# melspectrum007/audio-visual-speech-enhancement

Measured on AMD Instinct MI355X. Metric: clips/sec (STFT+CNN forward) on 200-ms@16kHz segments, 1/2/4/8 MI355X, higher is better.
Workload: dtype fp32_split

## Files before the change

### audio-visual-speech-enhancement_amd/csrc/avse_common.h

```cpp
#pragma once
#include <hip/hip_runtime.h>
#include <stdint.h>
#include <string>

#include "forward_plan.h"
#include "ragged_geom.h"

typedef __bf16 bf16_t;
typedef __bf16 bf16x8 __attribute__((ext_vector_type(8)));
typedef _Float16 f16x8 __attribute__((ext_vector_type(8)));
typedef _Float16 f16x4 __attribute__((ext_vector_type(4)));
typedef float f32x4 __attribute__((ext_vector_type(4)));
typedef int i32x4 __attribute__((ext_vector_type(4)));

struct avse_ctx;

namespace avse {

void set_error(const std::string& msg);

int ctx_device_index(const struct ::avse_ctx* c);

int ensure_lds_attr(const void* fn, int bytes);

// ... 98 lines not shown
    int N;
    int hop;
    int n_mels;
    const float* pinvT;
    const float2* twiddle;
    const float* window;
    float* frames;
    float* sig;
    const float4* bins;
    const float* gram_inv;
};

int launch_istft(const IstftArgs& a, hipStream_t s);

int istft_ragged_chunk(int N, int hop, int n_mels, bool fused_tables);
int launch_istft_ragged(const IstftArgs& a, const RaggedGeom& g, const RaggedDev& d, hipStream_t s);

struct ConvArgs {
    const void* in;
    void* out;
    const void* w;
    const float* scale;
    const float* shift;
    const int2* taps;
    int N;
    int Hi, Wi, Ci;
    long long in_clip_stride;
    int Hq, Wq;
    int sy, sx;
    int oys, oxs;
    int Ho, Wo, Co;
    long long out_clip_stride;
    int out_pix_stride;
    int out_c_off;
    int pool;
    int act;
    int nphase;
    int ksplit;
    int ksplit_slabs;
    float* partial;
    const float* fuse_w;
    float fuse_bias;
    float* fuse_out;
    int out_s16;
    unsigned* range_flag;
    unsigned range_bit, range_in_bit;
    ConvPhase ph[MAX_PHASES];
};

__device__ __forceinline__ bool pair_out_of_range(float x) { return !(__builtin_fabsf(x) < 65520.f); }
__device__ __forceinline__ void range_report(unsigned* flag, unsigned bit, bool bad) {
    if (bad && flag) atomicOr(flag, bit);
}
constexpr unsigned kRangeAudioIn = 1u << 24, kRangeVideoIn = 1u << 25;
int launch_flag_or(unsigned* flag, unsigned bits, hipStream_t s);

constexpr int kConvSplit = 2, kConvSplitPairs = 3;
int launch_conv(const ConvArgs& a, int dtype, hipStream_t s);

int launch_conv_win(const ConvArgs& a, const int2* htaps, hipStream_t s);

struct DecTailArgs {
    const bf16_t* in;
    float* out;
    int N;
    const bf16_t* w4;
    const float* sc4;
    const float* sh4;
    int nt4, kpad4;
    int pt4, pl4, rows4, pitch4;
    int dy4, dx4, nx4;
    const bf16_t* w5;
    const float* sc5;
    const float* sh5;
    int nt5[4], kpad5[4];
    int dy5[4], dx5[4], nx5[4];
    long long woff5[4];
    int pt5, pl5, rows5, pitch5;
    const float* w6;
    float b6;
    unsigned* range_flag;
    unsigned range_bit;
    int four_products;
};
bool dec_tail_supported(const DecTailArgs& a);
bool dec_tail_s16_supported(const DecTailArgs& a);
int launch_dec_tail_s16(const DecTailArgs& a, hipStream_t s);

struct AudEncArgs {
    const float* mel;
    bf16_t* out;
    long long out_clip_stride;
    int N;
    const bf16_t* w1;
    const bf16_t* w2;
    const bf16_t* w3;
    const bf16_t* w4;
    const bf16_t* w5;
    const float* sc[5];
    const float* sh[5];
};
bool aud_enc_supported(const AudEncArgs& a);

struct DecHeadArgs {
    const bf16_t* in;
    long long in_clip_stride;
    bf16_t* out;
    long long out_clip_stride;
    int N;
    const bf16_t* w1;
    const bf16_t* w2;
    const bf16_t* w3;
    const float* sc[3];
    const float* sh[3];
};
bool dec_head_supported(const DecHeadArgs& a);
int launch_dec_head(const DecHeadArgs& a, hipStream_t s);

struct GemmArgs {
    const bf16_t* a;
    long long lda;
    const bf16_t* w;
    int M, N, kpad;
    const float* scale;
    const float* shift;
    int act;
    bf16_t* out;
    long long ldo;
    int out_off;
    int ksplit;
    float* partial;
    int* counters;
    int split;
    int slabs_per_split;
    unsigned* range_flag;
    unsigned range_bit;
    int counters_cap;
    int four_products;
};
int launch_gemm(const GemmArgs& g, int mode, hipStream_t s);
int launch_aud_enc(const AudEncArgs& a, hipStream_t s);
int launch_dec_tail(const DecTailArgs& a, hipStream_t s);

enum HaloOut { OUT_BF16 = 0, OUT_S16 = 1, OUT_F32 = 2 };

struct HaloArgs {
    int variant;
    const void* in;
    const float* video;
    const float* vmean;
    const float* vstd;
    void* out;
    const void* w;
    const float* scale;
    const float* shift;
    int N, Hc, Wc, Ci, Co;
    long long out_clip_stride;
    int out_pix_stride;
    int out_c_off;
    int mfma32;
    int no_planar;
    int split;
    int out_mode;
    unsigned long long* prof;
    unsigned* range_flag;
    unsigned range_bit, range_in_bit;
// ... 49 lines not shown
```

### audio-visual-speech-enhancement_amd/csrc/capi.hip

```cpp
#include <algorithm>
#include <cmath>
#include <cstdlib>
#include <cstring>
#include <mutex>
#include <set>

#include "ctx.h"
#include "eval_tables.h"
#include "spec_tables.h"

namespace avse {
static thread_local std::string g_err;
void set_error(const std::string& msg) { g_err = msg; }

int ensure_lds_attr(const void* fn, int bytes) {
    static std::mutex mu;
    static std::set<std::pair<const void*, int>> done;
    int dev = 0;
    AVSE_HIP_CHECK(hipGetDevice(&dev));
    std::lock_guard<std::mutex> lock(mu);
    if (done.count({fn, dev})) return 0;
    AVSE_HIP_CHECK(hipFuncSetAttribute(fn, hipFuncAttributeMaxDynamicSharedMemorySize, bytes));
    done.insert({fn, dev});
    return 0;
}

int fail(int code, const std::string& msg) {
    set_error(msg);
    return code;
}

int ctx_device_index(const avse_ctx* c) { return c->device; }
}

using namespace avse;

static_assert(sizeof(Cplx) == sizeof(float2) && offsetof(Cplx, im) == offsetof(float2, y), "Cplx must match float2");
static_assert(sizeof(MelBin) == sizeof(float4) && offsetof(MelBin, j0) == offsetof(float4, z), "MelBin must match float4");

struct OptionName {
    const char* name;
    const char* env;
    int Options::*field;
};
const OptionName kOptionNames[] = {
    {"no_gemm", "AVSE_NO_GEMM", &Options::no_gemm},
    {"no_audenc", "AVSE_NO_AUDENC", &Options::no_audenc},
    {"no_dechead", "AVSE_NO_DECHEAD", &Options::no_dechead},
    {"no_dectail", "AVSE_NO_DECTAIL", &Options::no_dectail},
    {"unfused_tail", "AVSE_UNFUSED_TAIL", &Options::unfused_tail},
    {"no_halo", "AVSE_NO_HALO", &Options::no_halo},
    {"mfma32", "AVSE_MFMA32", &Options::mfma32},
    {"serial", "AVSE_SERIAL", &Options::serial},
    {"graph", "AVSE_GRAPH", &Options::graph},
    {"gemm_ksplit_cap", "AVSE_GEMM_KSPLIT", &Options::gemm_ksplit_cap},
    {"dense_istft", "AVSE_DENSE_ISTFT", &Options::dense_istft},
    {"no_act_scale", "AVSE_NO_ACT_SCALE", &Options::no_act_scale},
    {"no_win", "AVSE_NO_WIN", &Options::no_win},
    {"no_v1p", "AVSE_NO_V1P", &Options::no_v1p},
    {"no_a1valu", "AVSE_NO_A1VALU", &Options::no_a1valu},
    {"no_planar", "AVSE_NO_PLANAR", &Options::no_planar},
    {"four_products", "AVSE_FOUR_PRODUCTS", &Options::four_products},
    {"side_prio", "AVSE_SIDE_PRIO", &Options::side_prio},
};

namespace {

const OptionName* find_option(const char* name) {
    for (const OptionName& o : kOptionNames)
        if (std::strcmp(o.name, name) == 0) return &o;
    return nullptr;
}

int upload_ragged(avse_ctx* c, const RaggedGeom& g, hipStream_t s, RaggedDev* d) {
    const size_t ub = sizeof(RaggedUtt) * g.utt.size(), ib = sizeof(RaggedItem) * g.items.size();
    const size_t need = ub + ib;
    hipStreamCaptureStatus cs = hipStreamCaptureStatusNone;
    if (s) AVSE_HIP_CHECK(hipStreamIsCapturing(s, &cs));
    const bool capturing = cs != hipStreamCaptureStatusNone;
    if (int rc = grow(c->prep, need, s, "preprocess scratch")) return rc;
    if (!capturing && c->ragged_done) AVSE_HIP_CHECK(hipEventSynchronize(c->ragged_done));
    if (int rc = grow(c->ragged_host, need, s, "ragged tables")) return rc;
    if (!c->ragged_done) AVSE_HIP_CHECK(hipEventCreateWithFlags(&c->ragged_done, hipEventDisableTiming));
    std::memcpy(c->ragged_host, g.utt.data(), ub);
    std::memcpy(c->ragged_host + ub, g.items.data(), ib);
    AVSE_HIP_CHECK(hipMemcpyAsync(c->prep, c->ragged_host, need, hipMemcpyHostToDevice, s));
    if (!capturing) AVSE_HIP_CHECK(hipEventRecord(c->ragged_done, s));
    d->utt = reinterpret_cast<const RaggedUtt*>(c->prep.p.get());
    d->items = reinterpret_cast<const RaggedItem*>(c->prep + ub);
    d->n_utt = (int)g.utt.size();
    d->n_items = (int)g.items.size();
    return 0;
}

template <typename D, typename T>
int table_to_device(const std::vector<T>& h, Owned<D>& out) {
    static_assert(sizeof(D) == sizeof(T), "element layout");
    AVSE_HIP_CHECK(out.alloc(sizeof(T) * h.size()));
    AVSE_HIP_CHECK(hipMemcpy(out, h.data(), sizeof(T) * h.size(), hipMemcpyHostToDevice));
    return 0;
}

int ensure_spec_tables(avse_ctx* c, int sr, int n_fft, int n_mels, double fmin, double fmax) {
    return build_spec_tables(c->spec, sr, n_fft, n_mels, fmin, fmax);
}

int ensure_istft_tables(avse_ctx* c, int sr, int n_fft, int n_mels, double fmin, double fmax) {
    return build_istft_tables(c->istft, sr, n_fft, n_mels, fmin, fmax);
}

int ensure_eval_tables(avse_ctx* c, int sr, bool any_rate, hipStream_t s, const EvalTables** out) {
    int up, down;
    eval_ratio(sr, &up, &down);
    const bool big = any_rate && std::max(up, down) > kEvalMaxRatio;
    for (const EvalTables& have : c->eval)
        if (have.sr == sr && have.big == big) {
            *out = &have;
            return 0;
        }
    if (int rc = not_capturing(s, "the tables of this sample rate would be built while the stream is being captured: run "
                                  "one call with this rate before the capture"))
        return rc;
    EvalTables& t = c->eval[c->eval_next];
    c->eval_next = (c->eval_next + 1) % 4;
    *out = &t;
    t = EvalTables();
    const int win = seg_snr_window(sr);
    const bool stoi = big || std::max(up, down) <= kEvalMaxRatio;
    const std::vector<double> taps = stoi ? resample_taps(up, down) : resample_taps(1, 1);
    if (big) {
        if (int rc = table_to_device(resample_taps_by_phase(taps, up), t.ptaps)) return rc;
    } else {
        if (int rc = table_to_device(taps, t.taps)) return rc;
    }
    if (int rc = table_to_device(hann_inner(kStoiFrame), t.W)) return rc;
    if (int rc = table_to_device(stoi_twiddle(), t.twid)) return rc;
    if (int rc = table_to_device(hann_inner(win), t.segw)) return rc;
    if (int rc = table_to_device(stoi_bands(), t.bands)) return rc;
    t.up = up; t.down = down; t.H = ((int)taps.size() - 1) / 2; t.win = win;
    t.sr = sr;
    t.big = big;
    return 0;
}

int spec_check(bool pointers, int64_t n_utt, const int64_t* n_samples, int sr, int n_fft, int hop, int n_mels, int pad_mode,
// ... 380 lines not shown
```

### audio-visual-speech-enhancement_amd/csrc/conv_dects.hip

```cpp
#include <cstdlib>
#include <utility>

#include "avse_common.h"

namespace avse {
namespace {

#ifndef AVSE_DECTS_ABL
#define AVSE_DECTS_ABL 0
#endif
constexpr int DABL = AVSE_DECTS_ABL;
constexpr float LRELU = 0.3f;
constexpr int kOOB = 0x7fffff00;
constexpr int H = 40, W = 10;
constexpr int CI4 = 128, CO = 64;
constexpr int NW = 8, NT = 64 * NW;
constexpr int R4 = 21;
constexpr int F4 = 14, F5 = 13, SL = 7;
constexpr int P4 = 18, S4 = 96, ROWS4 = 26, WBUF = ROWS4 * P4 * S4;
constexpr int LROWS4 = 24, LCOLS4 = 14, NPC = 3;
constexpr int P5 = 18, S5 = 288, ROWS5 = 23, OIMG = ROWS5 * P5 * S5;
constexpr int REGION = ((OIMG > 2 * WBUF ? OIMG : 2 * WBUF) + 1023) / 1024 * 1024;
constexpr int BOFF = REGION;
constexpr int PAR = BOFF + 2 * 4 * 4096;
// ... 352 lines not shown
            const int q = 16 * (fr0 + i) + r16;
            if (kg == 0 && q < H / 2 * W) xp[cb * (16 * F5) + q] = d;
        }
        lds_barrier();
        if (tid < H / 2 * W) {
            const int q = tid, yl = q / W, x = q - yl * W;
            const float v = ((xp[q] + xp[16 * F5 + q]) + xp[32 * F5 + q]) + xp[48 * F5 + q];
            outc[(2 * (H / 2 * half + yl) + py) * (2 * W) + 2 * x + px] = v + a.b6;
        }
        zero_all();
    };

    i32x2 pb[4];
    {
        i32x2 w0[4];
        unroll(std::make_integer_sequence<int, 4>{}, [&](auto tt) {
            constexpr int t = decltype(tt)::value;
            w0[t] = bpiece5(tt);
            pb[t] = bpiece5(std::integral_constant<int, t + 4>{});
        });
#pragma unroll
        for (int t = 0; t < 4; ++t) st8(bst + t * 4096, w0[t]);
    }
    zero_all();
    lds_barrier();
    i32x4 fa[2][SL], fl[SL], fw[2][2];
    read_a5(std::integral_constant<int, 0>{}, fa[0]);
    if constexpr (PR) read_a5p(std::integral_constant<int, 0>{}, kL, fl);
    read_w(0, fw[0]);
    if constexpr (PR) unroll(std::make_integer_sequence<int, ph_gstart(4) / 2>{}, [&](auto uu) {
        constexpr int u = decltype(uu)::value, g = 2 * u, p = ph_of(g);
        constexpr bool last = g + 2 == ph_gstart(p + 1);
        __builtin_amdgcn_sched_barrier(0);
        unroll(std::make_integer_sequence<int, 2>{}, [&](auto dd) {
            constexpr int gq = g + decltype(dd)::value;
            st8(bst + (((gq / 4) + 1) & 1) * 16384 + (gq % 4) * 4096, pb[gq & 3]);
            pb[gq & 3] = bpiece5(std::integral_constant<int, gq + 8>{});
        });
        if constexpr (g % 4 == 2) loop_barrier();
        if constexpr (!last && !(DABL & 2)) {
            read_a5p(std::integral_constant<int, g + 2>{}, kH, fa[(u + 1) & 1]);
            read_w((((g + 2) / 4) & 1) * 16384 + ((g + 2) % 4) * 4096, fw[(u + 1) & 1]);
        }
        __builtin_amdgcn_sched_barrier(0);
        mfma_l(fl, fw[u & 1], s6);
        __builtin_amdgcn_sched_barrier(0);
        if constexpr (!last && !(DABL & 2)) read_a5p(std::integral_constant<int, g + 2>{}, kL, fl);
        __builtin_amdgcn_sched_barrier(0);
        mfma_h(fa[u & 1], fw[u & 1], s6);
        if constexpr (!last && (g - ph_gstart(p)) % 8 == 6) flush();
        if constexpr (last) {
            epilogue5(std::integral_constant<int, p>{});
            if constexpr (p < 3) {
                read_a5p(std::integral_constant<int, g + 2>{}, kH, fa[(u + 1) & 1]);
                read_a5p(std::integral_constant<int, g + 2>{}, kL, fl);
                read_w((((g + 2) / 4) & 1) * 16384 + ((g + 2) % 4) * 4096, fw[(u + 1) & 1]);
            }
        }
    });
    else unroll(std::make_integer_sequence<int, ph_gstart(4)>{}, [&](auto gg) {
        constexpr int g = decltype(gg)::value, p = ph_of(g);
        constexpr bool last = g + 1 == ph_gstart(p + 1);
        __builtin_amdgcn_sched_barrier(0);
        st8(bst + (((g / 4) + 1) & 1) * 16384 + (g % 4) * 4096, pb[g & 3]);
        pb[g & 3] = bpiece5(std::integral_constant<int, g + 8>{});
        if constexpr (g % 4 == 3) loop_barrier();
        if constexpr (!last && !(DABL & 2)) {
            read_a5(std::integral_constant<int, g + 1>{}, fa[(g + 1) & 1]);
            read_w((((g + 1) / 4) & 1) * 16384 + ((g + 1) % 4) * 4096, fw[(g + 1) & 1]);
        }
        __builtin_amdgcn_sched_barrier(0);
        mfma_all(fa[g & 1], fw[g & 1], s6);
        if constexpr (!last && (g - ph_gstart(p)) % 8 == 7) flush();
        if constexpr (last) {
            epilogue5(std::integral_constant<int, p>{});
            if constexpr (p < 3) {
                read_a5(std::integral_constant<int, g + 1>{}, fa[(g + 1) & 1]);
                read_w((((g + 1) / 4) & 1) * 16384 + ((g + 1) % 4) * 4096, fw[(g + 1) & 1]);
            }
        }
    });
}

}

bool dec_tail_s16_supported(const DecTailArgs& a) {
    if (a.N <= 0 || a.nt4 != 16 || a.kpad4 != 16 * CI4 || a.dy4 != 1 || a.dx4 != 1 || a.nx4 != 4) return false;
    if (a.pt4 != 2 || a.pl4 != 2 || a.pt5 != 1 || a.pl5 != 1) return false;
    for (int p = 0; p < 4; ++p)
        if (a.nt5[p] != ph_nt(p) || a.kpad5[p] != ph_nt(p) * CO || a.dy5[p] != (p >> 1) || a.dx5[p] != (p & 1) ||
            a.nx5[p] != ph_nx(p) || a.woff5[p] != ph_woff(p))
            return false;
    return true;
}

int launch_dec_tail_s16(const DecTailArgs& a, hipStream_t s) {
    auto* const kf = a.four_products ? k_dec_tail_s16<false> : k_dec_tail_s16<true>;
    if (int rc = ensure_lds_attr((const void*)kf, LDS_BYTES)) return rc;
    hipLaunchKernelGGL(kf, dim3(2 * a.N), dim3(NT), LDS_BYTES, s, a);
    AVSE_HIP_CHECK(hipGetLastError());
    return 0;
}

}
```

### audio-visual-speech-enhancement_amd/csrc/forward.hip

```cpp
#include <algorithm>
#include <cstdio>
#include <cstring>

#include "ctx.h"

using namespace avse;

namespace {

HaloArgs halo_args(const GpuLayer& G, const void* in, const void* video, int video_dtype, const float* vmean,
                   const float* vstd, void* out, long long out_clip_stride, int out_pix_stride, int out_c_off, int64_t N,
                   const Options& opt) {
    HaloArgs a;
    std::memset(&a, 0, sizeof(a));
    a.variant = G.halo;
    a.in = in;
    a.video = reinterpret_cast<const float*>(video);
    a.video_u8 = video_dtype == AVSE_VIDEO_U8;
    a.vmean = vmean;
    a.vstd = vstd;
    a.out = out;
    a.w = G.w_halo;
    a.mfma32 = opt.mfma32;
    a.no_planar = opt.no_planar;
// ... 312 lines not shown
    }

    const bool concurrent = ev == nullptr && !opt.serial && !aud_fused;
    hipStream_t sa = s;
    if (concurrent) {
        if (!c->side) {
            if (opt.side_prio) {
                int least = 0, greatest = 0;
                AVSE_HIP_CHECK(hipDeviceGetStreamPriorityRange(&least, &greatest));
                AVSE_HIP_CHECK(hipStreamCreateWithPriority(&c->side, hipStreamNonBlocking, opt.side_prio == 1 ? least : greatest));
            } else {
                AVSE_HIP_CHECK(hipStreamCreateWithFlags(&c->side, hipStreamNonBlocking));
            }
            AVSE_HIP_CHECK(hipEventCreateWithFlags(&c->fork, hipEventDisableTiming));
            AVSE_HIP_CHECK(hipEventCreateWithFlags(&c->join, hipEventDisableTiming));
        }
        AVSE_HIP_CHECK(hipEventRecord(c->fork, s));
        AVSE_HIP_CHECK(hipStreamWaitEvent(c->side, c->fork, 0));
        sa = c->side;
    }
    if (aud_fused && ((rc = launch_aud_enc(aa, s)) || (rc = r.mark(6)))) return rc;
    const bool a1_valu = split && !aud_fused && !opt.no_a1valu && W->a1_valu_shape;
    if (a1_valu) {
        const GpuLayer& G = L(0);
        const int pt = std::max((G.ho - 1) * G.def.sh + G.def.kh - G.def.hin, 0) / 2;
        const int pl = std::max((G.wo - 1) * G.def.sw + G.def.kw - G.def.win, 0) / 2;
        if ((rc = r.mark()) ||
            (rc = launch_aconv1_split(audio, G.w_f32, G.scale, G.shift, buf(B_A1), N, G.def.hin, G.def.win, G.ho, G.wo,
                                      G.def.kh, G.def.kw, G.def.sh, pt, pl, G.def.cout, rflag, 1u, kRangeAudioIn, sa)) ||
            (rc = r.mark()))
            return rc;
    }
    if (!aud_fused && !a1_valu && ((rc = launch_audio_prep(audio, buf(B_AIN), N * kMels * P.T, gdt, sa)) || (rc = r.mark()))) return rc;
    const int a_in[5] = {B_AIN, B_A1, B_A2, B_A3, B_A4};
    for (int i = a1_valu ? 1 : 0; i < 5 && !aud_fused; ++i) {
        const GpuLayer& G = L(i);
        const long long in_cs = (long long)G.def.hin * G.def.win * (i == 0 ? G.cin_pad : G.def.cin);
        ConvArgs a = (i < 4) ? conv_args(G, buf(a_in[i]), in_cs, buf(a_in[i + 1]), (long long)G.ho * G.wo * G.def.cout, G.def.cout, 0, N)
                             : conv_args(G, buf(a_in[i]), in_cs, buf(B_CAT), CAT, G.def.cout, 0, N);
        const int dti = r.pairs(a, i > 0, true, i, rflag);
        if ((rc = r.conv(a, dti, G, sa)) || (rc = r.mark())) return rc;
    }
    if (concurrent) AVSE_HIP_CHECK(hipEventRecord(c->join, sa));
    if (video) {
        if ((rc = r.video_encoder(video, vdt, vmean, vstd, N, off, buf(B_CAT), rflag, true))) return rc;
    } else {
        const size_t es = r.es();
        if ((rc = launch_broadcast_row(W->vzero_emb.load(std::memory_order_acquire), (char*)buf(B_CAT) + AEMB * es, N, 2048 * es, CAT * es, s))) return rc;
        if (split && W->vzero_range && rflag && (rc = launch_flag_or(rflag, W->vzero_range, s))) return rc;
        if ((rc = r.mark(6))) return rc;
    }
    if (concurrent) AVSE_HIP_CHECK(hipStreamWaitEvent(s, c->join, 0));
    const struct { int li, in, out; long long lda, ldo; } dense[3] = {
        {11, B_CAT, B_E1, CAT, EMB}, {12, B_E1, B_E2, EMB, EMB}, {13, B_E2, B_E3, EMB, AEMB}};
    for (const auto& d : dense)
        if ((rc = r.gemm_layer(d.li, buf(d.in), d.lda, buf(d.out), d.ldo, (int)d.ldo, 0, N, off[B_COUNT], rflag)) || (rc = r.mark()))
            return rc;
    const int d_in[6] = {B_E3, B_D1, B_D2, B_D3, B_D4, B_D5};
    for (int i = 0; i < 5; ++i) {
        const GpuLayer& G = L(14 + i);
        const long long in_cs = (long long)G.def.hin * G.def.win * G.def.cin;
        if (i == 0 && dt == AVSE_BF16 && W->dec_head_shapes && !opt.no_dechead) {
            DecHeadArgs ha;
            std::memset(&ha, 0, sizeof(ha));
            ha.in = reinterpret_cast<const bf16_t*>(buf(B_E3));
            ha.in_clip_stride = AEMB;
            ha.out = reinterpret_cast<bf16_t*>(buf(B_D3));
            ha.out_clip_stride = 40 * 10 * 128;
            ha.N = (int)N;
            ha.w1 = (const bf16_t*)L(14).w; ha.w2 = (const bf16_t*)L(15).w; ha.w3 = (const bf16_t*)L(16).w;
            for (int k = 0; k < 3; ++k) { ha.sc[k] = L(14 + k).scale; ha.sh[k] = L(14 + k).shift; }
            if (dec_head_supported(ha)) {
                if ((rc = launch_dec_head(ha, s)) || (rc = r.mark(3))) return rc;
                i = 2;
                continue;
            }
        }
        if (i == 3 && dt != AVSE_F32 && !opt.unfused_tail && !opt.no_dectail) {
            DecTailArgs da = dec_tail_args(L(17), L(18), W, buf(d_in[3]), out, N);
            if (split) {
                da.range_flag = rflag;
                da.range_bit = 1u << 17;
                da.four_products = opt.four_products;
            }
            if (split ? dec_tail_s16_supported(da) : dec_tail_supported(da)) {
                if ((rc = split ? launch_dec_tail_s16(da, s) : launch_dec_tail(da, s)) || (rc = r.mark(2))) return rc;
                break;
            }
        }
        if (i == 4 && !opt.unfused_tail) {
            ConvArgs a = conv_args(G, buf(d_in[i]), in_cs, nullptr, (long long)G.ho * G.wo, 1, 0, N);
            a.fuse_w = W->d6_w;
            a.fuse_bias = W->d6_bias;
            a.fuse_out = out;
            const int dti = r.pairs(a, true, false, 14 + i, rflag);
            if ((rc = r.conv(a, dti, G, s)) || (rc = r.mark())) return rc;
            continue;
        }
        ConvArgs a = conv_args(G, buf(d_in[i]), in_cs, buf(d_in[i + 1]), (long long)G.ho * G.wo * G.def.cout, G.def.cout, 0, N);
        const int dti = r.pairs(a, true, i < 4 || !opt.unfused_tail, 14 + i, rflag);
        if ((rc = r.conv(a, dti, G, s)) || (rc = r.mark())) return rc;
    }
    if (opt.unfused_tail) {
        if ((rc = launch_out_conv(buf(B_D5), W->d6_w, W->d6_bias, out, N * kMels * P.T, gdt, s)) || (rc = r.mark())) return rc;
    } else if ((rc = r.mark())) {
        return rc;
    }
    return 0;
}

int forward_dispatch(avse_ctx* c, const avse_weights* W, const float* audio, const void* video, int vdt,
                     const float* vmean, const float* vstd, int64_t N, float* out, void* stream, unsigned* rflag) {
    if (!c || !W || N <= 0 || !c->opt.graph)
        return forward_impl(c, W, audio, video, vdt, vmean, vstd, N, out, (hipStream_t)stream, nullptr, rflag);
    AVSE_HIP_CHECK(hipSetDevice(c->device));
    if (W->device != c->device) return fail(AVSE_ERR_INVALID, "weights and context are on different devices");
    int rc = ensure_arena(c, N, W->dtype, W->shape, (hipStream_t)stream);
    if (rc) return rc;
    const void* key[10] = {(const void*)W->serial, audio, video, vmean, vstd, out, c->arena.p.get(), (const void*)c->arena.bytes,
                           rflag, (const void*)(uintptr_t)vdt};
    avse_ctx::Graph* hit = nullptr;
    for (auto& g : c->graphs)
        if (g.n == N && std::memcmp(&g.opt, &c->opt, sizeof(Options)) == 0 && std::memcmp(g.key, key, sizeof(key)) == 0)
            hit = &g;
    if (hit && hit->exec) {
        AVSE_HIP_CHECK(hipGraphLaunch(hit->exec, (hipStream_t)stream));
        return 0;
    }
    if (!hit) {
        if (c->graphs.size() >= 8) {
            if (c->graphs.front().exec) (void)hipGraphExecDestroy(c->graphs.front().exec);
            c->graphs.erase(c->graphs.begin());
        }
        avse_ctx::Graph g;
        std::memcpy(g.key, key, sizeof(key));
        g.n = N;
        g.opt = c->opt;
        g.exec = nullptr;
        c->graphs.push_back(g);
        return forward_impl(c, W, audio, video, vdt, vmean, vstd, N, out, (hipStream_t)stream, nullptr, rflag);
    }
    if (!c->cap) AVSE_HIP_CHECK(hipStreamCreateWithFlags(&c->cap, hipStreamNonBlocking));
    AVSE_HIP_CHECK(hipStreamBeginCapture(c->cap, hipStreamCaptureModeRelaxed));
    rc = forward_impl(c, W, audio, video, vdt, vmean, vstd, N, out, c->cap, nullptr, rflag);
    hipGraph_t graph = nullptr;
    const hipError_t ce = hipStreamEndCapture(c->cap, &graph);
    if (rc || ce != hipSuccess) {
        if (graph) (void)hipGraphDestroy(graph);
        return rc ? rc : fail(AVSE_ERR_HIP, std::string("forward capture: ") + hipGetErrorString(ce));
    }
    hipGraphExec_t exec = nullptr;
    const hipError_t ie = hipGraphInstantiate(&exec, graph, nullptr, nullptr, 0);
    (void)hipGraphDestroy(graph);
    if (ie != hipSuccess) return fail(AVSE_ERR_HIP, std::string("forward graph instantiate: ") + hipGetErrorString(ie));
    hit->exec = exec;
    AVSE_HIP_CHECK(hipGraphLaunch(exec, (hipStream_t)stream));
    return 0;
}

}

extern "C" {

int avse_ctx_reserve(avse_ctx* c, int64_t max_clips, int dtype) {
    if (!c || max_clips < 0 || !valid_dtype(dtype)) return fail(AVSE_ERR_INVALID, "bad reserve args");
    AVSE_HIP_CHECK(hipSetDevice(c->device));
// ... 124 lines not shown
```

### audio-visual-speech-enhancement_amd/csrc/options.h

```cpp
#pragma once

namespace avse {

struct Options {
    int no_gemm = 0;
    int no_audenc = 0;
    int no_dechead = 0;
    int no_dectail = 0;
    int unfused_tail = 0;
    int no_halo = 0;
    int mfma32 = 0;
    int serial = 0;
    int graph = 0;
    int gemm_ksplit_cap = 0;
    int dense_istft = 0;
    int no_act_scale = 0;
    int no_win = 0;
    int no_v1p = 0;
    int no_a1valu = 0;
    int no_planar = 0;
    int four_products = 0;
    int side_prio = 0;
};

enum HaloVariant { HALO_NONE = -1, HALO_V1 = 0, HALO_K5 = 1, HALO_K3_16 = 2, HALO_K3_8 = 3, HALO_V1P = 4 };

}
```

Baseline: 82460.

## Add warp-specialized fused decoder-tail kernel with dedicated loader waves

Adds a new split-fp16 decoder-tail kernel in which four waves issue MFMAs over two column blocks each (one pair on the leading row slice, one on the trailing slice) while the other four waves only stream input windows and weights from global memory into LDS rings. Compute waves run at raised priority and synchronise with loaders via per-ring-group barriers. It becomes the default path, with the old kernel kept behind a narrow option. The aim is to hide global-load latency behind matrix work, at the cost of fewer compute waves and more accumulator registers per wave.

```diff
diff --git a/audio-visual-speech-enhancement_amd/csrc/avse_common.h b/audio-visual-speech-enhancement_amd/csrc/avse_common.h
--- a/audio-visual-speech-enhancement_amd/csrc/avse_common.h
+++ b/audio-visual-speech-enhancement_amd/csrc/avse_common.h
@@ -204,6 +204,7 @@
     unsigned* range_flag;
     unsigned range_bit;
     int four_products;
+    int narrow;
 };
 bool dec_tail_supported(const DecTailArgs& a);
 bool dec_tail_s16_supported(const DecTailArgs& a);
diff --git a/audio-visual-speech-enhancement_amd/csrc/capi.hip b/audio-visual-speech-enhancement_amd/csrc/capi.hip
--- a/audio-visual-speech-enhancement_amd/csrc/capi.hip
+++ b/audio-visual-speech-enhancement_amd/csrc/capi.hip
@@ -61,6 +61,7 @@
     {"no_a1valu", "AVSE_NO_A1VALU", &Options::no_a1valu},
     {"no_planar", "AVSE_NO_PLANAR", &Options::no_planar},
     {"four_products", "AVSE_FOUR_PRODUCTS", &Options::four_products},
+    {"dectail_narrow", "AVSE_DECTAIL_NARROW", &Options::dectail_narrow},
     {"side_prio", "AVSE_SIDE_PRIO", &Options::side_prio},
 };
 
diff --git a/audio-visual-speech-enhancement_amd/csrc/conv_dects.hip b/audio-visual-speech-enhancement_amd/csrc/conv_dects.hip
--- a/audio-visual-speech-enhancement_amd/csrc/conv_dects.hip
+++ b/audio-visual-speech-enhancement_amd/csrc/conv_dects.hip
@@ -458,6 +458,425 @@
     });
 }
 
+constexpr int CW = 4, LT = NT - 64 * CW;
+constexpr int NPCL = (LROWS4 * LCOLS4 * 4 + LT - 1) / LT;
+constexpr int PSTL = 4;
+static_assert(LT == 256 && NPCL - 1 + PSTL < 16, "a chunk's window pieces are stored before the chunk's last barrier");
+constexpr bool d4_barrier(int t) { return t % 4 == 2; }
+constexpr bool d5_barrier(int g) { return g % 4 == 2; }
+constexpr bool d5_last(int g) { return g + 2 == ph_gstart(ph_of(g) + 1); }
+constexpr int wide_barriers() {
+    int n = 1;
+    for (int c = 0; c < 8; ++c)
+        for (int t = 0; t < 16; t += 2) n += d4_barrier(t);
+    n += 2;
+    for (int g = 0; g < ph_gstart(4); g += 2) n += d5_barrier(g) + d5_last(g);
+    return n;
+}
+static_assert(wide_barriers() == 1 + 8 * 4 + 2 + ph_gstart(4) / 4 + 4, "one barrier per ring group and phase epilogue");
+static_assert(d5_barrier(ph_gstart(1) - 2) && d5_barrier(ph_gstart(2) - 2) && d5_barrier(ph_gstart(3) - 2) &&
+                  d5_barrier(ph_gstart(4) - 2) && d4_barrier(14),
+              "a phase's (chunk's) last pair closes a ring group");
+
+template <bool LD, bool S6>
+__device__ __forceinline__ void dec_tail_wide(const DecTailArgs& a, char* const lds) {
+    const int tid = threadIdx.x, lane = tid & 63, lt = tid & (LT - 1);
+    const int w = __builtin_amdgcn_readfirstlane(tid >> 6) & (CW - 1);
+    const int r16 = lane & 15, kg = lane >> 4;
+    const int clip = blockIdx.x >> 1, half = blockIdx.x & 1;
+    const int cb0 = 2 * (w & 1);
+    constexpr int fr0 = S6 ? 0 : SL;
+    constexpr bool s6 = S6;
+
+    const int brow = lt >> 2, kq = lt & 3;
+    const int bst = BOFF + brow * 64 + ((kq ^ wsw(brow)) << 4);
+    const int brd = 16 * cb0 + r16, bps = (kg >> 1) * 4096;
+    const int bfh = BOFF + bps + brd * 64 + (((kg & 1) ^ wsw(brd)) << 4);
+    const int bfl = BOFF + bps + brd * 64 + (((2 + (kg & 1)) ^ wsw(brd)) << 4);
+    auto st16 = [&](int addr, i32x4 v) { *reinterpret_cast<i32x4*>(lds + addr) = v; };
+    auto read_w = [&](auto bb, int off, i32x4 (&f)[2]) {
+        constexpr int b = decltype(bb)::value;
+        f[0] = lds16(lds + b * 1024, bfh + off);
+        f[1] = lds16(lds + b * 1024, bfl + off);
+    };
+    constexpr std::integral_constant<int, 0> kB0{}, kH{};
+    constexpr std::integral_constant<int, 1> kB1{}, kL{};
+
+    f32x4 acc[2][SL], part[2][SL];
+    auto zero_all = [&]() {
+#pragma unroll
+        for (int b = 0; b < 2; ++b)
+#pragma unroll
+            for (int i = 0; i < SL; ++i) acc[b][i] = part[b][i] = (f32x4){0.f, 0.f, 0.f, 0.f};
+    };
+    auto flush = [&]() {
+#pragma unroll
+        for (int b = 0; b < 2; ++b)
+#pragma unroll
+            for (int i = 0; i < SL; ++i) {
+                acc[b][i] += part[b][i];
+                asm volatile("" : "+v"(acc[b][i]));
+                part[b][i] = (f32x4){0.f, 0.f, 0.f, 0.f};
+            }
+    };
+    auto mfma_l = [&](auto bb, int i, const i32x4& fl, const i32x4 (&fw)[2]) {
+        constexpr int b = decltype(bb)::value;
+        if constexpr (DABL & 1) {
+            asm volatile("" ::"v"(fl), "v"(fw[0]));
+            return;
+        }
+        part[b][i] = __builtin_amdgcn_mfma_f32_16x16x32_f16(__builtin_bit_cast(f16x8, fw[0]), __builtin_bit_cast(f16x8, fl),
+                                                            part[b][i], 0, 0, 0);
+    };
+    auto mfma_h = [&](auto bb, int i, const i32x4& fa, const i32x4 (&fw)[2]) {
+        constexpr int b = decltype(bb)::value;
+        if constexpr (DABL & 1) {
+            asm volatile("" ::"v"(fa), "v"(fw[0]), "v"(fw[1]));
+            return;
+        }
+        part[b][i] = __builtin_amdgcn_mfma_f32_16x16x32_f16(__builtin_bit_cast(f16x8, fw[0]), __builtin_bit_cast(f16x8, fa),
+                                                            part[b][i], 0, 0, 0);
+        part[b][i] = __builtin_amdgcn_mfma_f32_16x16x32_f16(__builtin_bit_cast(f16x8, fw[1]), __builtin_bit_cast(f16x8, fa),
+                                                            part[b][i], 0, 0, 0);
+    };
+    auto pair_l = [&](auto nn, const i32x4 (&fl)[SL], const i32x4 (&fw)[2][2], auto&& next_fa) {
+        constexpr int n = decltype(nn)::value;
+        unroll(std::make_integer_sequence<int, 2 * n>{}, [&](auto kk) {
+            constexpr int k = decltype(kk)::value, i = k % n;
+            if constexpr (k < n) mfma_l(kB0, i, fl[i], fw[0]);
+            else mfma_l(kB1, i, fl[i], fw[1]);
+            if constexpr (k % 2 == 1) next_fa(std::integral_constant<int, k / 2>{});
+            __builtin_amdgcn_sched_barrier(0);
+        });
+    };
+    auto pair_h = [&](auto nn, const i32x4 (&fa)[SL], const i32x4 (&fw)[2][2], auto&& next_fl, auto&& next_w) {
+        constexpr int n = decltype(nn)::value;
+        unroll(std::make_integer_sequence<int, n>{}, [&](auto ii) {
+            constexpr int i = decltype(ii)::value;
+            mfma_h(kB0, i, fa[i], fw[0]);
+            if constexpr (i < 4) next_fl(ii);
+            __builtin_amdgcn_sched_barrier(0);
+        });
+        next_w(kB0);
+        __builtin_amdgcn_sched_barrier(0);
+        unroll(std::make_integer_sequence<int, n>{}, [&](auto ii) {
+            constexpr int i = decltype(ii)::value;
+            mfma_h(kB1, i, fa[i], fw[1]);
+            if constexpr (i + 4 < n) next_fl(std::integral_constant<int, i + 4>{});
+            __builtin_amdgcn_sched_barrier(0);
+        });
+        next_w(kB1);
+        __builtin_amdgcn_sched_barrier(0);
+    };
+    auto loop_barrier_w = [&](auto young) {
+        if constexpr (DABL & 4) return;
+        if constexpr (LD) {
+            lds_barrier_raw();
+        } else {
+            asm volatile("s_waitcnt lgkmcnt(%0)" ::"n"(decltype(young)::value) : "memory");
+            asm volatile("s_barrier" ::: "memory");
+        }
+    };
+    constexpr std::integral_constant<int, SL> kAll{};
+    constexpr std::integral_constant<int, S6 ? SL : SL - 1> kN5{};
+    auto par4 = [&](int base, int cb) { return *reinterpret_cast<const f32x4*>(lds + base + (16 * cb + 4 * kg) * 4); };
+    constexpr auto ring_off = [](int s) { return ((s / 4) & 1) * 16384 + (s % 4) * 4096; };
+
+    const __amdgpu_buffer_rsrc_t rsW5 = make_rsrc(a.w5, (long long)ph_woff(4) * 4);
+    int vrow5[3];
+    vrow5[0] = brow * (4 * CO * 4) + kq * 16;
+    vrow5[1] = brow * (6 * CO * 4) + kq * 16;
+    vrow5[2] = brow * (9 * CO * 4) + kq * 16;
+    auto bpiece5 = [&](auto gg) {
+        constexpr int g = decltype(gg)::value < ph_gstart(4) ? decltype(gg)::value : ph_gstart(3);
+        constexpr int p = ph_of(g), sl = g - ph_gstart(p);
+        constexpr int kk = p == 0 ? 0 : p == 3 ? 2 : 1;
+        return __builtin_amdgcn_raw_buffer_load_b128(rsW5, vrow5[kk], ph_woff(p) * 4 + sl * 64, 0);
+    };
+    i32x4 pb[4];
+
+    const int r0 = 19 * half;
+    bool range_bad = false;
+    {
+        const long long in_clip = (long long)H * W * CI4 * 4;
+        const __amdgpu_buffer_rsrc_t rsIn = make_rsrc(reinterpret_cast<const char*>(a.in) + clip * in_clip, in_clip);
+        int psrc[NPCL], pdst[NPCL];
+        bool pok[NPCL];
+#pragma unroll
+        for (int k = 0; k < NPCL; ++k) {
+            const int p = (lt >> 2) + (LT / 4) * k, sg = lt & 3;
+            const int wr = p / LCOLS4, wc = p - wr * LCOLS4;
+            const int iy = r0 - 2 + wr, ix = wc - 2;
+            pok[k] = p < LROWS4 * LCOLS4;
+            const bool in = pok[k] && iy >= 0 && iy < H && ix >= 0 && ix < W;
+            psrc[k] = in ? ((iy * W + ix) * CI4 * 2 + sg * 8) * 2 : kOOB;
+            pdst[k] = (wr * P4 + wc) * S4 + sg * 16;
+        }
+        const __amdgpu_buffer_rsrc_t rsW = make_rsrc(a.w4, (long long)CO * 16 * CI4 * 4);
+        const int vbl = brow * (16 * CI4 * 4) + kq * 16;
+        auto bpiece = [&](auto tt, int csoff) {
+            constexpr int t = decltype(tt)::value;
+            return __builtin_amdgcn_raw_buffer_load_b128(rsW, vbl + t * 512, csoff, 0);
+        };
+        int vb[SL];
+#pragma unroll
+        for (int i = 0; i < SL; ++i) {
+            const int q = 16 * (fr0 + i) + r16, r = q / W, x = q - r * W;
+            vb[i] = (r * P4 + x) * S4 + (kg & 1) * 16 - (kg >> 1) * S4;
+        }
+        auto read_ap1 = [&](auto tt, auto hl, int wo, int i) {
+            constexpr int t = decltype(tt)::value % 16;
+            constexpr int imm = ((3 - t / 4) * P4 + (3 - t % 4)) * S4 + 32 * decltype(hl)::value;
+            return lds16(lds + imm + wo, vb[i]);
+        };
+        auto read_ap = [&](auto tt, auto hl, int wo, i32x4 (&f)[SL]) {
+#pragma unroll
+            for (int i = 0; i < SL; ++i) f[i] = read_ap1(tt, hl, wo, i);
+        };
+        if constexpr (LD) {
+            i32x4 pc[NPCL], w0[4];
+#pragma unroll
+            for (int k = 0; k < NPCL; ++k) pc[k] = __builtin_amdgcn_raw_buffer_load_b128(rsIn, psrc[k], 0, 0);
+            unroll(std::make_integer_sequence<int, 4>{}, [&](auto tt) {
+                constexpr int t = decltype(tt)::value;
+                w0[t] = bpiece(tt, 0);
+                pb[t] = bpiece(std::integral_constant<int, t + 4>{}, 0);
+            });
+#pragma unroll
+            for (int k = 0; k < NPCL; ++k)
+                if (pok[k]) st16(pdst[k], pc[k]);
+#pragma unroll
+            for (int t = 0; t < 4; ++t) st16(bst + t * 4096, w0[t]);
+        } else {
+            zero_all();
+        }
+        lds_barrier();
+
+        i32x4 fa[2][SL], fl[SL], fw[2][2];
+        i32x4 pr[NPCL];
+        int wb = 0;
+        if constexpr (!LD) {
+            read_ap(std::integral_constant<int, 0>{}, kH, 0, fa[0]);
+            read_ap(std::integral_constant<int, 0>{}, kL, 0, fl);
+            read_w(kB0, 0, fw[0]);
+            read_w(kB1, 0, fw[1]);
+        }
+        for (int c = 0; c < 8; ++c) {
+            const int nb = (c & 1) ? 0 : WBUF;
+            const int cs = c * 64, cn = (c + 1) * 64;
+            unroll(std::make_integer_sequence<int, 8>{}, [&](auto uu) {
+                constexpr int u = decltype(uu)::value, t = 2 * u;
+                __builtin_amdgcn_sched_barrier(0);
+                if constexpr (LD) {
+                    unroll(std::make_integer_sequence<int, 2>{}, [&](auto dd) {
+                        constexpr int tq = t + decltype(dd)::value;
+                        st16(bst + ring_off(tq + 4), pb[tq & 3]);
+                        if constexpr (tq + 8 < 16) pb[tq & 3] = bpiece(std::integral_constant<int, tq + 8>{}, cs);
+                        else if (c < 7) pb[tq & 3] = bpiece(std::integral_constant<int, tq + 8 - 16>{}, cn);
+                        else pb[tq & 3] = bpiece5(std::integral_constant<int, tq - 8>{});
+                        if constexpr (tq < NPCL) pr[tq] = __builtin_amdgcn_raw_buffer_load_b128(rsIn, psrc[tq], cn, 0);
+                        if constexpr (tq >= PSTL && tq - PSTL < NPCL) {
+                            if (pok[tq - PSTL] && c < 7) st16(nb + pdst[tq - PSTL], pr[tq - PSTL]);
+                        }
+                    });
+                } else {
+                    pair_l(kAll, fl, fw, [&](auto ii) {
+                        constexpr int i = decltype(ii)::value;
+                        if constexpr (DABL & 2) {
+                        } else if constexpr (t < 14) {
+                            fa[(u + 1) & 1][i] = read_ap1(std::integral_constant<int, t + 2>{}, kH, wb, i);
+                        } else if (c < 7) {
+                            fa[0][i] = read_ap1(std::integral_constant<int, 0>{}, kH, nb, i);
+                        }
+                    });
+                }
+                if constexpr (d4_barrier(t)) loop_barrier_w(std::integral_constant<int, (DABL & 2) ? 0 : SL>{});
+                if constexpr (!LD) {
+                    pair_h(kAll, fa[u & 1], fw,
+                           [&](auto ii) {
+                               constexpr int i = decltype(ii)::value;
+                               if constexpr (DABL & 2) {
+                               } else if constexpr (t < 14) {
+                                   fl[i] = read_ap1(std::integral_constant<int, t + 2>{}, kL, wb, i);
+                               } else if (c < 7) {
+                                   fl[i] = read_ap1(std::integral_constant<int, 0>{}, kL, nb, i);
+                               }
+                           },
+                           [&](auto bb) {
+                               if constexpr (!(DABL & 2)) read_w(bb, ring_off(t + 2), fw[decltype(bb)::value]);
+                           });
+                    if constexpr (t % 8 == 6) flush();
+                }
+                if constexpr (t == 14) wb = nb;
+            });
+        }
+        lds_barrier();
+
+        if constexpr (LD) {
+            const int zrow = half ? 21 : 0;
+            for (int u = lt; u < (12 + 2 * 22) * 16; u += LT) {
+                const int px = u >> 4, pc = u & 15;
+                const int i = px < 12 ? zrow : (px - 12) >> 1, xi = px < 12 ? px : ((px - 12) & 1) * 11;
+                st16((i * P5 + xi) * S5 + pc * 16, (i32x4){0, 0, 0, 0});
+            }
+        } else {
+            int lane4 = lane;
+            asm volatile("" : "+v"(lane4));
+#pragma unroll
+            for (int b = 0; b < 2; ++b) {
+                const int cb = cb0 + b;
+                const f32x4 sc = par4(PSC4, cb), sh = par4(PSH4, cb);
+#pragma unroll
+                for (int i = 0; i < SL; ++i) {
+                    const int q = 16 * (fr0 + i) + (lane4 & 15);
+                    if (q >= R4 * W) continue;
+                    const int r = q / W, x = q - r * W;
+                    const int px = ((r + 1 - half) * P5 + x + 1) * S5 + cb * 64 + 8 * (lane4 >> 4);
+                    f16x4 hv, lv;
+#pragma unroll
+                    for (int e = 0; e < 4; ++e) {
+                        const float y = bn_lrelu(acc[b][i][e], sc[e], sh[e]);
+                        range_bad |= pair_out_of_range(y);
+                        hv[e] = (_Float16)y;
+                        lv[e] = (_Float16)(y - (float)hv[e]);
+                    }
+                    *reinterpret_cast<f16x4*>(lds + px) = hv;
+                    *reinterpret_cast<f16x4*>(lds + px + 32) = lv;
+                }
+            }
+        }
+        lds_barrier();
+    }
+    if constexpr (!LD) range_report(a.range_flag, a.range_bit, range_bad);
+
+    float* const outc = a.out + (long long)clip * (4 * H * W);
+    int tid5 = tid;
+    asm volatile("" : "+v"(tid5));
+    const int r16_5 = tid5 & 15, kg_5 = (tid5 >> 4) & 3;
+    int vb5[SL];
+#pragma unroll
+    for (int i = 0; i < SL; ++i) {
+        const int q = 16 * (fr0 + i) + r16_5, yl = q / W, x = q - yl * W;
+        vb5[i] = (yl * P5 + x) * S5 + (kg_5 & 1) * 16 + (kg_5 >> 1) * 64;
+    }
+    auto read_a5p1 = [&](auto gg, auto hl, int i) {
+        constexpr int g = decltype(gg)::value;
+        constexpr int p = ph_of(g), sl = g - ph_gstart(p), tap = sl / 4, c = sl % 4;
+        static_assert(c % 2 == 0, "a pair lies inside one tap");
+        constexpr int dy = (p >> 1) - tap / ph_nx(p), dx = (p & 1) - tap % ph_nx(p);
+        constexpr int imm = ((dy + 1) * P5 + (dx + 1)) * S5 + c * 64 + 32 * decltype(hl)::value;
+        return lds16(lds + imm, vb5[i]);
+    };
+    auto read_a5p = [&](auto gg, auto hl, i32x4 (&f)[SL]) {
+#pragma unroll
+        for (int i = 0; i < (s6 ? SL : SL - 1); ++i) f[i] = read_a5p1(gg, hl, i);
+    };
+    float* const xp = reinterpret_cast<float*>(lds + XP);
+    auto epilogue5 = [&](auto pp) {
+        constexpr int p = decltype(pp)::value, py = p >> 1, px = p & 1;
+        if constexpr (!LD) {
+            constexpr int n = s6 ? SL : SL - 1;
+            flush();
+            float d[2][SL];
+#pragma unroll
+            for (int b = 0; b < 2; ++b) {
+                const f32x4 sc = par4(PSC5, cb0 + b), sh = par4(PSH5, cb0 + b), w6 = par4(PW6, cb0 + b);
+#pragma unroll
+                for (int i = 0; i < n; ++i) {
+                    d[b][i] = 0.f;
+#pragma unroll
+                    for (int e = 0; e < 4; ++e) d[b][i] = fmaf(bn_lrelu(acc[b][i][e], sc[e], sh[e]), w6[e], d[b][i]);
+                }
+            }
+#pragma unroll
+            for (int k = 0; k < 2 * n; ++k) d[k / n][k % n] += __shfl_xor(d[k / n][k % n], 16);
+#pragma unroll
+            for (int k = 0; k < 2 * n; ++k) d[k / n][k % n] += __shfl_xor(d[k / n][k % n], 32);
+            if (kg == 0) {
+#pragma unroll
+                for (int k = 0; k < 2 * n; ++k) {
+                    const int q = 16 * (fr0 + k % n) + r16;
+                    if (q < H / 2 * W) xp[(cb0 + k / n) * (16 * F5) + q] = d[k / n][k % n];
+                }
+            }
+        }
+        lds_barrier();
+        if constexpr (LD) {
+            if (lt < H / 2 * W) {
+                const int q = lt, yl = q / W, x = q - yl * W;
+                const float v = ((xp[q] + xp[16 * F5 + q]) + xp[32 * F5 + q]) + xp[48 * F5 + q];
+                outc[(2 * (H / 2 * half + yl) + py) * (2 * W) + 2 * x + px] = v + a.b6;
+            }
+        } else {
+            zero_all();
+        }
+    };
+
+    if constexpr (!LD) zero_all();
+    i32x4 fa[2][SL], fl[SL], fw[2][2];
+    auto read_pair5 = [&](auto gg, i32x4 (&fh)[SL]) {
+        constexpr int g = decltype(gg)::value;
+        read_a5p(gg, kH, fh);
+        read_a5p(gg, kL, fl);
+        read_w(kB0, ring_off(g), fw[0]);
+        read_w(kB1, ring_off(g), fw[1]);
+    };
+    if constexpr (!LD) read_pair5(std::integral_constant<int, 0>{}, fa[0]);
+    unroll(std::make_integer_sequence<int, ph_gstart(4) / 2>{}, [&](auto uu) {
+        constexpr int u = decltype(uu)::value, g = 2 * u, p = ph_of(g);
+        constexpr bool last = d5_last(g), ahead = !last && !(DABL & 2);
+        __builtin_amdgcn_sched_barrier(0);
+        if constexpr (LD) {
+            unroll(std::make_integer_sequence<int, 2>{}, [&](auto dd) {
+                constexpr int gq = g + decltype(dd)::value;
+                st16(bst + ring_off(gq + 4), pb[gq & 3]);
+                pb[gq & 3] = bpiece5(std::integral_constant<int, gq + 8>{});
+            });
+        } else {
+            pair_l(kN5, fl, fw, [&](auto ii) {
+                if constexpr (ahead) fa[(u + 1) & 1][decltype(ii)::value] = read_a5p1(std::integral_constant<int, g + 2>{}, kH, decltype(ii)::value);
+            });
+        }
+        if constexpr (d5_barrier(g)) loop_barrier_w(std::integral_constant<int, ahead ? (S6 ? SL : SL - 1) : 0>{});
+        if constexpr (!LD) {
+            pair_h(kN5, fa[u & 1], fw,
+                   [&](auto ii) {
+                       if constexpr (ahead) fl[decltype(ii)::value] = read_a5p1(std::integral_constant<int, g + 2>{}, kL, decltype(ii)::value);
+                   },
+                   [&](auto bb) {
+                       if constexpr (ahead) read_w(bb, ring_off(g + 2), fw[decltype(bb)::value]);
+                   });
+            if constexpr (!last && (g - ph_gstart(p)) % 8 == 6) flush();
+        }
+        if constexpr (last) {
+            epilogue5(std::integral_constant<int, p>{});
+            if constexpr (p < 3 && !LD) read_pair5(std::integral_constant<int, g + 2>{}, fa[(u + 1) & 1]);
+        }
+    });
+}
+
+__global__ __launch_bounds__(NT, 1) void k_dec_tail_s16w(DecTailArgs a) {
+    extern __shared__ __attribute__((aligned(1024))) char lds[];
+    const int tid = threadIdx.x;
+    if (tid < 64) {
+        reinterpret_cast<float*>(lds + PSC4)[tid] = a.sc4[tid];
+        reinterpret_cast<float*>(lds + PSH4)[tid] = a.sh4[tid];
+        reinterpret_cast<float*>(lds + PSC5)[tid] = a.sc5[tid];
+        reinterpret_cast<float*>(lds + PSH5)[tid] = a.sh5[tid];
+        reinterpret_cast<float*>(lds + PW6)[tid] = a.w6[tid];
+    }
+    const int wave = __builtin_amdgcn_readfirstlane(tid >> 6);
+    if (wave < CW / 2) {
+        __builtin_amdgcn_s_setprio(2);
+        dec_tail_wide<false, true>(a, lds);
+    } else if (wave < CW) {
+        __builtin_amdgcn_s_setprio(2);
+        dec_tail_wide<false, false>(a, lds);
+    } else {
+        dec_tail_wide<true, false>(a, lds);
+    }
+}
+
 }
 
 bool dec_tail_s16_supported(const DecTailArgs& a) {
@@ -471,7 +890,7 @@
 }
 
 int launch_dec_tail_s16(const DecTailArgs& a, hipStream_t s) {
-    auto* const kf = a.four_products ? k_dec_tail_s16<false> : k_dec_tail_s16<true>;
+    auto* const kf = a.four_products ? k_dec_tail_s16<false> : a.narrow ? k_dec_tail_s16<true> : k_dec_tail_s16w;
     if (int rc = ensure_lds_attr((const void*)kf, LDS_BYTES)) return rc;
     hipLaunchKernelGGL(kf, dim3(2 * a.N), dim3(NT), LDS_BYTES, s, a);
     AVSE_HIP_CHECK(hipGetLastError());
diff --git a/audio-visual-speech-enhancement_amd/csrc/forward.hip b/audio-visual-speech-enhancement_amd/csrc/forward.hip
--- a/audio-visual-speech-enhancement_amd/csrc/forward.hip
+++ b/audio-visual-speech-enhancement_amd/csrc/forward.hip
@@ -418,6 +418,7 @@
                 da.range_flag = rflag;
                 da.range_bit = 1u << 17;
                 da.four_products = opt.four_products;
+                da.narrow = opt.dectail_narrow;
             }
             if (split ? dec_tail_s16_supported(da) : dec_tail_supported(da)) {
                 if ((rc = split ? launch_dec_tail_s16(da, s) : launch_dec_tail(da, s)) || (rc = r.mark(2))) return rc;
diff --git a/audio-visual-speech-enhancement_amd/csrc/options.h b/audio-visual-speech-enhancement_amd/csrc/options.h
--- a/audio-visual-speech-enhancement_amd/csrc/options.h
+++ b/audio-visual-speech-enhancement_amd/csrc/options.h
@@ -20,6 +20,7 @@
     int no_a1valu = 0;
     int no_planar = 0;
     int four_products = 0;
+    int dectail_narrow = 0;
     int side_prio = 0;
 };
 
```

Result: no change. 83240, median of 6 (+0.9%).
